# openai/robogym

Measured on AMD Instinct MI355X. Metric: env-steps/sec (whole node) dactyl/locked batch 8192; qpos L∞ vs MuJoCo (as restated by the in-repo CPU oracle: parity unpinned), higher is better.
Workload: dtype f32

## Files before the change

### robogym_amd/csrc/rg_kernel.h

```cpp
#ifndef RG_KERNEL_COMMON_H
#define RG_KERNEL_COMMON_H
#include "rg_types.h"

#ifdef RG_EMUL
#include "hip_emul.h"
#else
#include <hip/hip_runtime.h>
#endif

#ifdef RG_EMUL
typedef const RgModelDev& RgM;
#else
typedef const __attribute__((address_space(4))) RgModelDev& RgM;
#endif
#ifdef RG_FINE_PROF
#define RG_NPROF 56
#else
#define RG_NPROF 24
#endif
struct RgAux {
  const int *subtree_adr, *subtree;
  const uint32_t* dof_velmask;
};

// ... 446 lines not shown
    PFOR(d, m.nv) {
      float xf = 0;
      for (int b = 1; b < m.nbody; b++) {
        if (!in_chain(m, b, d)) continue;
        const float* w = P + RG_PRM_XFRC + 6 * b;
        v3 off = rg_xipos(m, s, b) - ld3(s.org + 3 * s.b2org[b]);
        xf += dot(ld3(w), jac_col(s, d, off)) + dot(ld3(w + 3), ld3(s.cdof + 6 * d));
      }
      s.qfrc_smooth[d] = xf;
    }
    SYNC();
  }
}


__device__ __forceinline__ bool seg_intersect(float p1x, float p1y, float p2x, float p2y, float p3x, float p3y, float p4x, float p4y) {
  float det = (p4y - p3y) * (p2x - p1x) - (p4x - p3x) * (p2y - p1y);
  if (fabsf(det) < 1e-15f) return false;
  float idet = rg_rcp(det);
  float a = ((p4x - p3x) * (p1y - p3y) - (p4y - p3y) * (p1x - p3x)) * idet;
  float b = ((p2x - p1x) * (p1y - p3y) - (p2y - p1y) * (p1x - p3x)) * idet;
  return a >= 0 && a <= 1 && b >= 0 && b <= 1;
}
__device__ __forceinline__ float wrap_circle(float* pnt, const float* d, bool has_sd, float sd0, float sd1, float rad) {
  float sq0 = d[0] * d[0] + d[1] * d[1], sq1 = d[2] * d[2] + d[3] * d[3], sqr = rad * rad;
  float dx = d[2] - d[0], dy = d[3] - d[1], dd = dx * dx + dy * dy;
  if (sq0 < sqr || sq1 < sqr || rad < 1e-15f || dd < 1e-15f) return -1;
  float a = clampf(-(dx * d[0] + dy * d[1]) * rg_rcp(dd), 0.f, 1.f);
  float nx = a * dx + d[0], ny = a * dy + d[1];
  if (nx * nx + ny * ny > sqr && (!has_sd || sd0 * nx + sd1 * ny >= 0)) return -1;
  float sol[2][4], good[2];
  float r0 = rg_sqrt(sq0 - sqr), r1 = rg_sqrt(sq1 - sqr), isq0 = rg_rcp(sq0), isq1 = rg_rcp(sq1);
  for (int i = 0; i < 2; i++) {
    float sgn = i == 0 ? 1.f : -1.f;
    sol[i][0] = (d[0] * sqr + sgn * rad * d[1] * r0) * isq0; sol[i][1] = (d[1] * sqr - sgn * rad * d[0] * r0) * isq0;
    sol[i][2] = (d[2] * sqr - sgn * rad * d[3] * r1) * isq1; sol[i][3] = (d[3] * sqr + sgn * rad * d[2] * r1) * isq1;
    if (has_sd) {
      float mx = sol[i][0] + sol[i][2], my = sol[i][1] + sol[i][3], n = fmaxf(rg_sqrt(mx * mx + my * my), 1e-15f);
      good[i] = (mx * sd0 + my * sd1) * rg_rcp(n);
    } else {
      float tx = sol[i][0] - sol[i][2], ty = sol[i][1] - sol[i][3];
      good[i] = -(tx * tx + ty * ty);
    }
    if (seg_intersect(d[0], d[1], sol[i][0], sol[i][1], d[2], d[3], sol[i][2], sol[i][3])) good[i] = -10000.f;
  }
  int k = good[0] > good[1] ? 0 : 1;
  for (int e = 0; e < 4; e++) pnt[e] = sol[k][e];
  if (seg_intersect(d[0], d[1], pnt[0], pnt[1], d[2], d[3], pnt[2], pnt[3])) return -1;
  return rad * acosf(clampf((pnt[0] * pnt[2] + pnt[1] * pnt[3]) * rg_rcp(sqr), -1.f, 1.f));
}
__device__ __forceinline__ float rg_wrap(v3& w0, v3& w1, v3 x0, v3 x1, v3 gpos, const float* gmat, float radius, int type, bool has_side, v3 side) {
  v3 p0 = mulmT(gmat, x0 - gpos), p1 = mulmT(gmat, x1 - gpos);
  if (norm(p0) < 1e-15f || norm(p1) < 1e-15f) return -1;
  v3 ax0, ax1;
  if (type == RG_WRAP_SPHERE) {
    ax0 = normalized(p0);
    v3 nrm = cross(p0, p1);
    if (norm(nrm) < 1e-15f) nrm = cross(ax0, fabsf(ax0.x) < 0.9f ? mk3(1, 0, 0) : mk3(0, 1, 0));
    nrm = normalized(nrm); ax1 = normalized(cross(nrm, ax0));
  } else { ax0 = mk3(1, 0, 0); ax1 = mk3(0, 1, 0); }
  float dd[4] = {dot(p0, ax0), dot(p0, ax1), dot(p1, ax0), dot(p1, ax1)}, sd0 = 0, sd1 = 0;
  if (has_side) {
    v3 sl = mulmT(gmat, side - gpos);
    sd0 = dot(sl, ax0); sd1 = dot(sl, ax1);
    float n = fmaxf(rg_sqrt(sd0 * sd0 + sd1 * sd1), 1e-15f), rn = radius * rg_rcp(n);
    sd0 *= rn; sd1 *= rn;
  }
  float pnt[4], wlen = wrap_circle(pnt, dd, has_side, sd0, sd1, radius);
  if (wlen < 0) return -1;
  v3 r0 = ax0 * pnt[0] + ax1 * pnt[1], r1 = ax0 * pnt[2] + ax1 * pnt[3];
  if (type == RG_WRAP_CYLINDER) {
    float L0 = rg_sqrt((dd[0] - pnt[0]) * (dd[0] - pnt[0]) + (dd[1] - pnt[1]) * (dd[1] - pnt[1]));
    float L1 = rg_sqrt((dd[2] - pnt[2]) * (dd[2] - pnt[2]) + (dd[3] - pnt[3]) * (dd[3] - pnt[3]));
    float iL = rg_rcp(L0 + wlen + L1);
    r0.z = p0.z + (p1.z - p0.z) * L0 * iL;
    r1.z = p0.z + (p1.z - p0.z) * (L0 + wlen) * iL;
    wlen = rg_sqrt(wlen * wlen + (r1.z - r0.z) * (r1.z - r0.z));
  }
  w0 = mulm(gmat, r0) + gpos; w1 = mulm(gmat, r1) + gpos;
  return wlen;
}

__device__ __forceinline__ void rg_tendon(RgM m, RgLds& s) {
  PFOR(t, m.ntendon) {
    int r0 = m.ten_path_adr[t], r1 = m.ten_path_adr[t + 1];
    const int* td = m.ten_dofs + 4 * t;
    int d0 = td[0], d1 = td[1], d2 = td[2], d3 = td[3];
    float J[4] = {0, 0, 0, 0}, L = 0;
    for (int r = r0; r < r1; r++) {
      const rgf4* R = (const rgf4*)m.ten_path + 2 * r;
      rgf4 ra = R[0], rb = R[1];
      int kind = __builtin_bit_cast(int, ra.x), w1 = __builtin_bit_cast(int, ra.y), w2 = __builtin_bit_cast(int, ra.z);
      if ((kind & 15) == 0) {
        float coef = ra.w;
        L += coef * s.qpos[w1];
        for (int e = 0; e < 4; e++) if (e == w2) J[e] += coef;
        continue;
      }
      float idiv = ra.w, radius = rb.x; int bits = __builtin_bit_cast(int, rb.y);
      int s0 = w1 & 255, s1 = (w1 >> 8) & 255, g = (w1 >> 16) & 255, sid = (w1 >> 24) & 255;
      int ba = w2 & 255, bs = (w2 >> 8) & 255, bg = (w2 >> 16) & 255;
      v3 pa = ld3(s.spos + 3 * s0), x1 = ld3(s.spos + 3 * s1), pb = x1, pc = mk3(0, 0, 0), pd = mk3(0, 0, 0);
      bool two = false;
      float wlen = -1;
      if ((kind & 15) == 2) {
        v3 w0 = mk3(0, 0, 0), w1p = mk3(0, 0, 0);
        float gm[9]; q2mat(gm, ldq(s.gquat + 4 * g));
        wlen = rg_wrap(w0, w1p, pa, x1, ld3(s.gpos + 3 * g), gm, radius, kind >> 4, sid != 255, sid != 255 ? ld3(s.spos + 3 * sid) : mk3(0, 0, 0));
        if (wlen >= 0) { pb = w0; pc = w1p; pd = x1; two = true; L += wlen * idiv; }
      }
      for (int seg = 0; seg < (two ? 2 : 1); seg++) {
        v3 q0 = seg ? pc : pa, q1 = seg ? pd : pb;
        int k0 = seg ? 2 : 0, k1 = two ? (seg ? 1 : 2) : 1;
        int b0 = seg ? bg : ba, b1 = two ? (seg ? bs : bg) : bs;
        v3 dif = q1 - q0;
        float dist = rg_sqrt(dot(dif, dif));
        L += dist * idiv;
        if (b0 != b1 && dist > 1e-15f) {
          dif = dif * rg_rcp(dist);
          v3 o0 = q0 - ld3(s.org + 3 * s.b2org[b0]), o1 = q1 - ld3(s.org + 3 * s.b2org[b1]);
          for (int e = 0; e < 4; e++) {
            int d = e == 0 ? d0 : (e == 1 ? d1 : (e == 2 ? d2 : d3));
            if (d < 0) continue;
            float v = 0;
            if ((bits >> (3 * e + k1)) & 1) v += dot(dif, jac_col(s, d, o1));
            if ((bits >> (3 * e + k0)) & 1) v -= dot(dif, jac_col(s, d, o0));
            J[e] += v * idiv;
          }
        }
      }
    }
    s.tenlen[t] = L;
    for (int e = 0; e < 4; e++) s.tenJ[4 * t + e] = J[e];
  }
  SYNC();
  PFOR(u, m.nu) {
    int id = m.actuator_trnid[u];
    s.actlen[u] = m.actuator_gear[u] * (m.actuator_trntype[u] == 0 ? s.qpos[m.jnt_qposadr[id]] : s.tenlen[id]);
  }
  SYNC();
}

__device__ __forceinline__ void rg_crb(RgM m, RgLds& s, const float* P, const int* subtree_adr, const int* subtree) {
  for (int w = LANE; w < m.nbody * 10; w += RG_WAVE) {
    int b = w / 10, k = w - 10 * b;
    float acc = 0;
    for (uint32_t bits = (uint32_t)m.subtree_mask[b]; bits; bits &= bits - 1) acc += s.cinert[10 * __builtin_ctz(bits) + k];
    s.crb[w] = acc;
  }
  SYNC();
  PFOR(e, m.nM) {
    const int ijb = m.M_ijb[e], i = ijb & 255, j = (ijb >> 8) & 255;
    float buf[6];
    mul_inert_vec(buf, s.crb + 10 * (ijb >> 16), s.cdof + 6 * i);
    const float* c = s.cdof + 6 * j;
    float v = c[0] * buf[0] + c[1] * buf[1] + c[2] * buf[2] + c[3] * buf[3] + c[4] * buf[4] + c[5] * buf[5];
    if (i == j) v += P[RG_PRM_DOF_ARMATURE + i];
    s.Msp[e] = v;
  }
  SYNC();
}
__device__ __forceinline__ void rg_M_to_blocks(RgM m, RgLds& s) {
  { rgf4 z; z.x = z.y = z.z = z.w = 0.f; rgf4* H4 = (rgf4*)s.H; for (int w = LANE; w < ((m.blkwords + 3) >> 2); w += RG_WAVE) H4[w] = z; }
  SYNC();
  PFOR(e, m.nM) { int a = m.M_ent[2 * e]; float v = s.Msp[e]; s.H[a & 0xFFFF] = v; s.H[(a >> 16) & 0xFFFF] = v; }
  SYNC();
}

struct SupPt { v3 v, s; };
struct MprGeom { int type; const float* quat; v3 pos; v3 size; int vertadr, nvert, mesh; float margin; float vscale = 1.f; };
struct MprEnv { const float* mesh_vert; const int* cell_adr; const rgf4 *cell_blk, *cell_ovf; float* prof; bool cells; bool plane_depth; };

__device__ __forceinline__ float vdot(v3 d, const rgf4& a) { return __builtin_fmaf(d.z, a.z, __builtin_fmaf(d.y, a.y, d.x * a.x)); }
template <int G> __device__ __forceinline__ void scan_batch(const rgf4* vert, int nvert, int base, v3 ld, float& bv, int& bi, v3& bp) {
  int i0 = base + (LANE & (G - 1)), last = nvert - 1;
  int j0 = i0 < last ? i0 : last, j1 = i0 + G < last ? i0 + G : last, j2 = i0 + 2 * G < last ? i0 + 2 * G : last, j3 = i0 + 3 * G < last ? i0 + 3 * G : last;
  rgf4 a = vert[j0], b = vert[j1], c = vert[j2], d = vert[j3];
  float da = vdot(ld, a), db = vdot(ld, b), dc = vdot(ld, c), dd = vdot(ld, d);
  if (da > bv) { bv = da; bi = j0; bp = mk3(a.x, a.y, a.z); }
  if (db > bv) { bv = db; bi = j1; bp = mk3(b.x, b.y, b.z); }
  if (dc > bv) { bv = dc; bi = j2; bp = mk3(c.x, c.y, c.z); }
  if (dd > bv) { bv = dd; bi = j3; bp = mk3(d.x, d.y, d.z); }
}
template <int G> __device__ __forceinline__ void scan_verts(const rgf4* vert, int nvert, v3 ld, float& bv, int& bi, v3& bp) {
  for (int base = 0; base < nvert; base += 4 * G) scan_batch<G>(vert, nvert, base, ld, bv, bi, bp);
}
__device__ __forceinline__ int dir_cell(v3 ld) {
  float ax = fabsf(ld.x), ay = fabsf(ld.y), az = fabsf(ld.z);
  int axis = ax >= ay ? (ax >= az ? 0 : 2) : (ay >= az ? 1 : 2);
  float mj = axis == 0 ? ld.x : (axis == 1 ? ld.y : ld.z), a = axis == 0 ? ld.y : (axis == 1 ? ld.z : ld.x), b = axis == 0 ? ld.z : (axis == 1 ? ld.x : ld.y);
  float inv = (0.5f * RG_CELLN) * rg_rcp(fmaxf(fabsf(mj), 1e-30f));
  int iu = (int)(a * inv + 0.5f * RG_CELLN), iv = (int)(b * inv + 0.5f * RG_CELLN);
  iu = iu < 0 ? 0 : (iu > RG_CELLN - 1 ? RG_CELLN - 1 : iu); iv = iv < 0 ? 0 : (iv > RG_CELLN - 1 ? RG_CELLN - 1 : iv);
  return ((2 * axis + (mj < 0 ? 1 : 0)) * RG_CELLN + iu) * RG_CELLN + iv;
}
template <int G> __device__ __forceinline__ void scan_cell(const int* celladr, const rgf4* cellblk, const rgf4* cellovf, v3 ld, float& bv, int& bi, v3& bp) {
  int cell = dir_cell(ld), l = LANE & (G - 1);
  int e = celladr[cell];
  if (G >= 4) {
    rgf4 a = cellblk[4 * cell + (l & 3)];
    float da = vdot(ld, a);
    if (da > bv) { bv = da; bi = __builtin_bit_cast(int, a.w); bp = mk3(a.x, a.y, a.z); }
  } else {
    rgf4 a = cellblk[4 * cell + 2 * (l & 1)], a2 = cellblk[4 * cell + 2 * (l & 1) + 1];
    float da = vdot(ld, a), da2 = vdot(ld, a2);
    if (da > bv) { bv = da; bi = __builtin_bit_cast(int, a.w); bp = mk3(a.x, a.y, a.z); }
    int i2 = __builtin_bit_cast(int, a2.w);
    if (da2 > bv || (da2 == bv && i2 < bi)) { bv = da2; bi = i2; bp = mk3(a2.x, a2.y, a2.z); }
  }
  int cnt = (e & 255) - 4, last = cnt - 1;
  if (cnt > 0) {
    const rgf4* rec = cellovf + (e >> 8);
    for (int base = 0; base < cnt; base += 2 * G) {
      int i0 = base + l, j0 = i0 < last ? i0 : last, j1 = i0 + G < last ? i0 + G : last;
      rgf4 b = rec[j0], c = rec[j1];
      float db = vdot(ld, b), dc = vdot(ld, c);
      int ib = __builtin_bit_cast(int, b.w), ic = __builtin_bit_cast(int, c.w);
      if (db > bv || (db == bv && ib < bi)) { bv = db; bi = ib; bp = mk3(b.x, b.y, b.z); }
      if (dc > bv || (dc == bv && ic < bi)) { bv = dc; bi = ic; bp = mk3(c.x, c.y, c.z); }
    }
  }
}
template <int G> __device__ __forceinline__ void scan_hull(const MprEnv& E, const MprGeom& g, v3 ld, float& bv, int& bi, v3& bp) {
  if (E.cells) scan_cell<G>(E.cell_adr + g.mesh * RG_NCELL, E.cell_blk + (size_t)g.mesh * (RG_NCELL * 4), E.cell_ovf, ld, bv, bi, bp);
  else scan_verts<G>((const rgf4*)E.mesh_vert + g.vertadr, g.nvert, ld, bv, bi, bp);
}
template <int G> __device__ __forceinline__ v3 pick_vert(float bv, int bi, v3 bp) {
  if (G == 64) {
    float vm = wave_max(bv);
    int wi = wave_min_i(bv == vm ? bi : 0x7fffffff);
    int wl = wave_min_i((bv == vm && bi == wi) ? LANE : 0x7fffffff);
    return mk3(lane_bcast(bp.x, wl), lane_bcast(bp.y, wl), lane_bcast(bp.z, wl));
  } else {
    float vm = grp_max<G>(bv);
    int wi = grp_min_i<G>(bv == vm ? bi : 0x7fffffff);
    bool win = bv == vm && bi == wi;
    return mk3(grp_max<G>(win ? bp.x : -3.0e38f), grp_max<G>(win ? bp.y : -3.0e38f), grp_max<G>(win ? bp.z : -3.0e38f));
  }
}
__device__ __forceinline__ v3 support_primitive(const MprGeom& g, v3 ld) {
// ... 496 lines not shown
        const float sc1 = (hdr & RG_PAIR_SCALED1) ? gscale : 1.f, sc2 = (hdr & RG_PAIR_SCALED2) ? gscale : 1.f;
        r3.z *= sc1; r3.w *= sc2;
        v3 p1 = ld3(s.gpos + 3 * g1), p2 = ld3(s.gpos + 3 * g2), dif = p2 - p1;
        isbb = ((hdr >> 20) & 255) == (RG_GEOM_BOX | (RG_GEOM_BOX << 4)); ispl = ((hdr >> 20) & 15) == RG_GEOM_PLANE;
        if (((hdr >> 20) & 15) == RG_GEOM_PLANE) {
          float d = dot(dif, qrot(ldq(s.gquat + 4 * g1), mk3(0, 0, 1))) - (r3.w + margin);
          hit = d <= 0; newlb = fmaxf(d, 0.f);
        } else {
          float d = sqrtf(dot(dif, dif)) - (r3.z + r3.w + margin);
          if (d <= 0) {
            float hm = 0.5f * margin + 1e-6f;
            v3 ea = mk3(r4.x * sc1 + hm, r4.y * sc1 + hm, r4.z * sc1 + hm), eb = mk3(r5.x * sc2 + hm, r5.y * sc2 + hm, r5.z * sc2 + hm);
            float Ra[9], Rb[9]; q2mat(Ra, ldq(s.gquat + 4 * g1)); q2mat(Rb, ldq(s.gquat + 4 * g2));
            float og = obb_gap(Ra, ea, Rb, eb, dif);
            hit = og < 0; newlb = fmaxf(og, 0.f);
          } else newlb = d;
        }
        if (pairlb) RG_ROW_ST(pairlb + q, fmaxf(newlb - 1e-6f, 0.f));
      }
      unsigned long long bal = __ballot(hit);
      bbany = bbany || (hit && isbb); plany = plany || (hit && ispl);
      int base = s.ncand;
      SYNC();
      if (hit) {
        int slot = base + __popcll(bal & ((1ull << LANE) - 1ull));
        if (slot < RG_MAXCAND) s.cand[slot] = q; else s.status |= RG_STATUS_CAND_FULL;
      }
      if (LANE == 0) { int n = base + __popcll(bal); s.ncand = n < RG_MAXCAND ? n : RG_MAXCAND; }
      SYNC();
    }
#ifdef RG_FINE_PROF
    if (prof && LANE == 0) prof[44] += (float)(rg_clock() - tref0);
#endif
    nt = 0;
  }
  if (prof && LANE == 0) prof[5] += (float)(rg_clock() - tb0);
  int ncand = s.ncand;
  if (LANE == 0) s.ncand2 = 0;
  SYNC();
  if (ncand > 16) rg_narrow_phase1<2>(c, ncand); else rg_narrow_phase1<4>(c, ncand);
  int ncand2 = s.ncand2;
  if (prof && LANE == 0) { prof[16] += (float)(rg_clock() - tb0); prof[17] += ncand; prof[18] += ncand2; }
  rg_narrow_phase2<4>(c, ncand2);
  if (prof && LANE == 0) prof[19] += (float)(rg_clock() - tb0);
  if (!(RG_L(c).flags & 16) && __ballot(bbany) != 0) rg_narrow_boxbox(c, ncand);
  if (__ballot(plany) != 0)
  for (int cbase = 0; cbase < ncand; cbase += RG_WAVE) {
  bool is_plane = false;
  if (cbase + LANE < ncand) is_plane = ((__builtin_bit_cast(int, m.pair_rec[RG_PAIRREC * s.cand[cbase + LANE]]) >> 20) & 15) == RG_GEOM_PLANE;
  unsigned long long plane_bits = __ballot(is_plane);
  while (plane_bits) {
    int ci = cbase + __builtin_ctzll(plane_bits); plane_bits &= plane_bits - 1;
    int p = s.cand[ci];
    int g1 = m.pair_geom[3 * p], g2 = m.pair_geom[3 * p + 1], dim = m.pair_geom[3 * p + 2];
    float margin = m.pair_prm[12 * p];
    int t2 = m.geom_type[g2];
    v3 p1 = ld3(s.gpos + 3 * g1), p2 = ld3(s.gpos + 3 * g2);
    MprGeom B;
    B.type = t2; B.quat = s.gquat + 4 * g2; B.size = ld3(m.geom_size + 3 * g2); B.margin = 0; B.mesh = -1; B.vertadr = 0; B.nvert = 0;
    if (__builtin_bit_cast(int, m.pair_rec[RG_PAIRREC * p]) & RG_PAIR_SCALED2) B.size = B.size * gscale;
    if (t2 == RG_GEOM_MESH) { B.mesh = m.geom_dataid[g2]; B.vertadr = m.mesh_vertadr[B.mesh]; B.nvert = m.mesh_vertnum[B.mesh]; }
    v3 n = qrot(ldq(s.gquat + 4 * g1), mk3(0, 0, 1));
    if (t2 == RG_GEOM_BOX) {
      int cnt = 0;
      for (int i = 0; i < 8 && cnt < 4; i++) {
        v3 lc = mk3((i & 1) ? B.size.x : -B.size.x, (i & 2) ? B.size.y : -B.size.y, (i & 4) ? B.size.z : -B.size.z);
        v3 c = qrot(ldq(B.quat), lc) + p2;
        float dist = dot(c - p1, n);
        if (dist > margin) continue;
        add_contact(s, p, dist, c - n * (0.5f * dist), n, dim); cnt++;
      }
    } else {
      B.pos = p2 - p1;
      v3 sp = rg_support<64>(rg_mpr_env(m, (float*)0, false), B, n * -1.0f);
      float dist = dot(sp, n);
      if (dist <= margin) add_contact(s, p, dist, sp + p1 - n * (0.5f * dist), n, dim);
    }
  }
  }
  SYNC();
}

__device__ __forceinline__ void rg_velocity(RgM m, RgLds& s, const float* P, const uint32_t* dof_velmask, const int* subtree_adr, const int* subtree) {
  PFOR(d, m.nv) {
    float cv[6] = {0, 0, 0, 0, 0, 0};
    for (int h = 0; h < 2; h++) {
      uint32_t bits = dof_velmask[2 * d + h];
      while (bits) { int a = __builtin_ctz(bits) + 32 * h; bits &= bits - 1; float q = s.qvel[a]; for (int e = 0; e < 6; e++) cv[e] += s.cdof[6 * a + e] * q; }
    }
    int j = m.dof_jntid[d];
    if (m.jnt_type[j] == RG_JNT_FREE && d - m.jnt_dofadr[j] < 3) { for (int e = 0; e < 6; e++) s.cdofdot[6 * d + e] = 0; }
    else cross_motion(s.cdofdot + 6 * d, cv, s.cdof + 6 * d);
  }
  PFOR(t, m.ntendon) {
    float v = 0;
    for (int e = 0; e < 4; e++) { int d = m.ten_dofs[4 * t + e]; if (d >= 0) v += s.tenJ[4 * t + e] * s.qvel[d]; }
    s.tenvel[t] = v;
    s.tenfrc[t] = m.tendon_stiffness[t] * (m.tendon_lengthspring[t] - s.tenlen[t]) - m.tendon_damping[t] * v;
  }
  SYNC();
  PFOR(k, m.body_geomnum[0]) s.gspeed[m.body_geomadr[0] + k] = 0;
  for (int b = 1 + LANE; b < m.nbody; b += RG_WAVE) {
    float cv[6] = {0, 0, 0, 0, 0, 0}, ca[6] = {0, 0, 0, -P[RG_PRM_GRAVITY], -P[RG_PRM_GRAVITY + 1], -P[RG_PRM_GRAVITY + 2]};
    for (int h = 0; h < 2; h++) {
      uint32_t bits = m.body_dofmask[2 * b + h];
      while (bits) {
        int a = __builtin_ctz(bits) + 32 * h; bits &= bits - 1; float q = s.qvel[a];
        for (int e = 0; e < 6; e++) { cv[e] += s.cdof[6 * a + e] * q; ca[e] += s.cdofdot[6 * a + e] * q; }
      }
    }
    {
      const float gsmax = fmaxf(P[RG_PRM_GEOM_SCALE], 1.f);
      v3 w = mk3(cv[0], cv[1], cv[2]), vo = mk3(cv[3], cv[4], cv[5]), og = ld3(s.org + 3 * s.b2org[b]);
      float wn = norm(w);
      int ga = m.body_geomadr[b], gn = m.body_geomnum[b];
      for (int k = 0; k < gn; k++) s.gspeed[ga + k] = norm(vo + cross(w, ld3(s.gpos + 3 * (ga + k)) - og)) + wn * (m.geom_rbound[ga + k] * gsmax);
    }
    float t1[6], t2[6], t3[6];
    mul_inert_vec(t1, s.cinert + 10 * b, ca);
    mul_inert_vec(t2, s.cinert + 10 * b, cv);
    cross_force(t3, cv, t2);
    for (int e = 0; e < 6; e++) s.cacc[6 * b + e] = t1[e] + t3[e];
  }
  SYNC();
  {
    float acc[(RG_MAXBODY * 6 + RG_WAVE - 1) / RG_WAVE];
#pragma unroll
    for (int k0 = 0; k0 < (RG_MAXBODY * 6 + RG_WAVE - 1) / RG_WAVE; k0++) {
      int w = LANE + RG_WAVE * k0, b = w / 6, k = w - 6 * b; float a = 0;
      if (w < m.nbody * 6 && b > 0) for (uint32_t bits = (uint32_t)m.subtree_mask[b]; bits; bits &= bits - 1) a += s.cacc[6 * __builtin_ctz(bits) + k];
      acc[k0] = a;
    }
    SYNC();
#pragma unroll
    for (int k0 = 0; k0 < (RG_MAXBODY * 6 + RG_WAVE - 1) / RG_WAVE; k0++) { int w = LANE + RG_WAVE * k0; if (w < m.nbody * 6) s.cacc[w] = acc[k0]; }
  }
  SYNC();
  PFOR(d, m.nv) {
    const rgf4 dr0 = ((const rgf4*)m.dof_rec)[2 * d]; const float spring_ref = m.dof_rec[8 * d + 4];
    const int w0 = __builtin_bit_cast(int, dr0.x);
    const float *c = s.cdof + 6 * d, *f = s.cacc + 6 * (w0 & 255);
    s.qfrc_bias[d] = c[0] * f[0] + c[1] * f[1] + c[2] * f[2] + c[3] * f[3] + c[4] * f[4] + c[5] * f[5];
    float pas = -P[RG_PRM_DOF_DAMPING + d] * s.qvel[d];
    if (dr0.z != 0) pas -= dr0.z * (s.qpos[__builtin_bit_cast(int, dr0.w)] - spring_ref);
    for (int q = (w0 >> 8) & 255; q < ((w0 >> 16) & 255); q++) { int tt = m.dof_ten[2 * q], sl = m.dof_ten[2 * q + 1]; pas += s.tenJ[4 * tt + sl] * s.tenfrc[tt]; }
    s.qfrc_passive[d] = pas;
  }
  SYNC();
}

static_assert(RG_MAXU <= RG_WAVE && RG_MAXNV <= RG_WAVE, "controller state / warm start: one lane per actuator / dof");
__device__ __forceinline__ void rg_pid(RgM m, RgLds& s, const float* P, float* st ) {
  float dt = P[RG_PRM_TIMESTEP];
  PFOR(u, m.nu) {
    const float* gp = P + RG_PRM_ACT_GAINPRM + 10 * u;
    float force;
    float lo = P[RG_PRM_ACT_FORCERANGE + 2 * u], hi = P[RG_PRM_ACT_FORCERANGE + 2 * u + 1];
    if (m.actuator_biastype[u] == 2) {
      float err = s.ctrl[u] - s.actlen[u];
      if (fabsf(err) < gp[5]) err = 0;
      float integ = clampf(st[0] + err * dt, -gp[2], gp[2]);
      float deriv = (1 - gp[4]) * st[2] + gp[4] * (err - st[1]) * rg_rcp(dt);
      force = gp[0] * (err + (gp[1] != 0 ? integ * rg_rcp(gp[1]) : 0.f) + gp[3] * deriv);
      st[0] = integ; st[1] = err; st[2] = deriv;
      if (lo != 0 || hi != 0) force = clampf(force, lo, hi);
    } else {
      float c = s.ctrl[u];
      if (m.actuator_ctrllimited[u]) c = clampf(c, P[RG_PRM_ACT_CTRLRANGE + 2 * u], P[RG_PRM_ACT_CTRLRANGE + 2 * u + 1]);
      force = gp[0] * c;
    }
    if (m.actuator_forcelimited[u]) force = clampf(force, lo, hi);
    s.actfrc[u] = force;
  }
  SYNC();
}
__device__ __forceinline__ void rg_smooth(RgM m, RgLds& s, const float* P) {
  PFOR(d, m.nv) {
    float f = 0;
    const int aw = __builtin_bit_cast(int, m.dof_rec[8 * d + 1]);
    for (int q = aw & 255; q < ((aw >> 8) & 255); q++) {
      int u = m.dof_act[2 * q], sl = m.dof_act[2 * q + 1];
      f += m.actuator_gear[u] * (sl < 0 ? 1.0f : s.tenJ[4 * m.actuator_trnid[u] + sl]) * s.actfrc[u];
    }
    s.qfrc_act[d] = f;
    float v = s.qfrc_passive[d] - s.qfrc_bias[d] + f + (s.has_xfrc ? s.qfrc_smooth[d] : 0.f);
    s.qfrc_smooth[d] = v; s.qacc_smooth[d] = v;
  }
  SYNC();
}

__device__ __forceinline__ float impedance(const float* si, float pos, float margin) {
  float dmin = clampf(si[0], 1e-4f, 0.9999f), dmax = clampf(si[1], 1e-4f, 0.9999f), width = fmaxf(si[2], 1e-15f);
  float mid = clampf(si[3], 1e-4f, 0.9999f), power = fmaxf(si[4], 1.0f);
  if (dmin == dmax || width <= 1e-15f) return 0.5f * (dmin + dmax);
  float x = fabsf((pos - margin) * rg_rcp(width));
  if (x >= 1) return dmax;
  if (x <= 0) return dmin;
  float y;
  if (power == 1) y = x;
  else if (power == 2) y = x <= mid ? x * x * rg_rcp(mid) : 1 - (1 - x) * (1 - x) * rg_rcp(1 - mid);
  else if (x <= mid) y = powf(x, power) / powf(mid, power - 1);
  else y = 1 - powf(1 - x, power) / powf(1 - mid, power - 1);
  return dmin + y * (dmax - dmin);
}
__device__ __forceinline__ void kb(float timestep, const float* solref, const float* solimp, float& K, float& B) {
  float dmax = clampf(solimp[1], 1e-4f, 0.9999f);
  if (solref[0] > 0) {
    float tc = fmaxf(solref[0], 2 * timestep), dr = solref[1];
    K = rg_rcp(fmaxf(1e-15f, dmax * dmax * tc * tc * dr * dr)); B = 2.0f * rg_rcp(fmaxf(1e-15f, dmax * tc));
  } else { K = -solref[0] / fmaxf(1e-15f, dmax * dmax); B = -solref[1] / fmaxf(1e-15f, dmax); }
}
__device__ __forceinline__ int nsrow(RgM m) { return m.nfric_dof + m.nfric_ten + 2 * m.nlim_jnt + 2 * m.nlim_ten; }
__device__ __forceinline__ void rg_build_row_desc(RgM m, RgLds& s) {
  int ns = nsrow(m);
  (void)ns;
  PFOR(w, m.ntendon * 4) { int d = m.ten_dofs[w]; s.ten_cdof[w] = (unsigned char)(d >= 0 ? m.d2c[d] : 255); }
  PFOR(i, m.nvc) { s.c2d[i] = (unsigned char)m.c2d[i]; s.cblk[i] = m.c_blk[i]; }
  PFOR(b, m.nbody) s.b2org[b] = (unsigned char)m.body_orgslot[b];
  SYNC();
}
template <bool FULL> __device__ __forceinline__ float srow_dot(const RgLds& s, int desc, const float* x) {
  int t = (desc >> 6) & 31; float v;
  if (t == 31) { int d = desc & 63; v = x[FULL ? s.c2d[d] : d]; }
  else { v = 0; for (int e = 0; e < 4; e++) { int d = s.ten_cdof[4 * t + e]; if (d != 255) v += s.tenJ[4 * t + e] * x[FULL ? s.c2d[d] : d]; } }
  return (desc >> 11) & 1 ? -v : v;
}
__device__ __forceinline__ void srow_scatter(RgLds& s, int desc, float coef, float* dst) {
  int t = (desc >> 6) & 31;
  if ((desc >> 11) & 1) coef = -coef;
  if (t == 31) { atomicAdd(dst + (desc & 63), coef); return; }
  for (int e = 0; e < 4; e++) { int d = s.ten_cdof[4 * t + e]; if (d != 255) atomicAdd(dst + d, coef * s.tenJ[4 * t + e]); }
}
__device__ __forceinline__ void srow_hess(RgM m, RgLds& s, int desc, float D) {
  int t = (desc >> 6) & 31;
  if (t == 31) { int d = desc & 63; atomicAdd(s.H + d * m.hs + d, D); return; }
  for (int a = 0; a < 4; a++) { int da = s.ten_cdof[4 * t + a]; if (da == 255) continue;
    for (int b = 0; b < 4; b++) { int db = s.ten_cdof[4 * t + b]; if (db == 255 || db > da) continue; atomicAdd(s.H + da * m.hs + db, D * s.tenJ[4 * t + a] * s.tenJ[4 * t + b]); } }
}
__device__ __forceinline__ void srow_hess_tree(RgLds& s, int desc, float D) {
  int t = (desc >> 6) & 31;
  if (t == 31) { int d = desc & 63, blk = s.cblk[d]; atomicAdd(s.H + (blk & 0xFFFF) + d - ((blk >> 16) & 255), D); return; }
  for (int a = 0; a < 4; a++) { int da = s.ten_cdof[4 * t + a]; if (da == 255) continue;
    int blk = s.cblk[da];
    for (int b = 0; b < 4; b++) { int db = s.ten_cdof[4 * t + b]; if (db == 255 || db > da) continue; atomicAdd(s.H + (blk & 0xFFFF) + db - ((blk >> 16) & 255), D * s.tenJ[4 * t + a] * s.tenJ[4 * t + b]); } }
}
__device__ __forceinline__ int npyr(int dim) { return dim == 1 ? 1 : 2 * (dim - 1); }
__device__ __forceinline__ int nbasis(int dim) { return dim >= 4 ? 4 : (dim == 1 ? 1 : 3); }

__device__ __forceinline__ void rg_make_constraint(RgM m, RgLds& s, const float* P) {
  int ncon = s.ncon;
  PFOR(c, ncon) {
    const float* R = m.pair_rec + RG_PAIRREC * s.c_pair[c];
    s.c_nnz[c] = __popc(__builtin_bit_cast(uint32_t, R[23])) + __popc(__builtin_bit_cast(uint32_t, R[24]));
  }
  SYNC();
  {
    int c = LANE, off = 0, sz = 0;
    if (c < ncon) { for (int q = 0; q < c; q++) off += nbasis(s.c_dim[q]) * s.c_nnz[q]; sz = nbasis(s.c_dim[c]) * s.c_nnz[c]; s.c_off[c] = off; }
#if defined(RG_CAP_HIST) && !defined(RG_EMUL)
    if (ncon > 0 && c == ncon - 1) { atomicAdd(rg_cap_hist + (ncon < 63 ? ncon : 63), 1u); const int bin = (off + sz) >> 4; atomicAdd(rg_cap_hist + 64 + (bin < 127 ? bin : 127), 1u); }
    if (ncon == 0 && c == 0) { atomicAdd(rg_cap_hist, 1u); atomicAdd(rg_cap_hist + 64, 1u); }
#endif
    int firstbad = wave_min_i((c < ncon && off + sz > RG_CPOOL) ? c : 0x7fffffff);
    if (firstbad < ncon) { ncon = firstbad; if (LANE == 0) { s.ncon = ncon; s.status |= RG_STATUS_CON_FULL; } }
  }
  SYNC();
  for (int w = LANE; w < ncon * RG_W; w += RG_WAVE) {
    int c = w / RG_W, sl = w - c * RG_W, p = s.c_pair[c], nnz = s.c_nnz[c];
    if (sl >= nnz) continue;
    const float* R = m.pair_rec + RG_PAIRREC * p;
    int bb = __builtin_bit_cast(int, R[19]), b1 = bb & 255, b2 = bb >> 8;
    uint32_t lo = __builtin_bit_cast(uint32_t, R[23]), hi = __builtin_bit_cast(uint32_t, R[24]);
    int k = sl; uint32_t bits = lo; int base = 0;
    if (k >= __popc(lo)) { k -= __popc(lo); bits = hi; base = 32; }
    for (int q = 0; q < k; q++) bits &= bits - 1;
    int d = base + __builtin_ctz(bits);
    v3 pos = ld3(s.c_pos + 3 * c);
    v3 jp = mk3(0, 0, 0), jr = mk3(0, 0, 0);
    if (in_chain(m, b2, d)) { jp = jp + jac_col(s, d, pos - ld3(s.org + 3 * s.b2org[b2])); jr = jr + ld3(s.cdof + 6 * d); }
    if (in_chain(m, b1, d)) { jp = jp - jac_col(s, d, pos - ld3(s.org + 3 * s.b2org[b1])); jr = jr - ld3(s.cdof + 6 * d); }
    float f[9]; st3(f, ld3(s.c_normal + 3 * c)); make_frame(f);
    s.c_idx[c * RG_W + sl] = (unsigned char)m.d2c[d];
    float* Bc = s.c_pool + s.c_off[c]; int nb = nbasis(s.c_dim[c]);
    Bc[sl] = dot(ld3(f), jp);
    if (nb >= 3) { Bc[nnz + sl] = dot(ld3(f + 3), jp); Bc[2 * nnz + sl] = dot(ld3(f + 6), jp); }
    if (nb >= 4) Bc[3 * nnz + sl] = dot(ld3(f), jr);
  }
  SYNC();
  PFOR(c, ncon) {
    int p = s.c_pair[c], dim = s.c_dim[c];
    const float* prm = m.pair_prm + 12 * p;
    const int hdr = __builtin_bit_cast(int, m.pair_rec[RG_PAIRREC * p]), bb = __builtin_bit_cast(int, m.pair_rec[RG_PAIRREC * p + 19]), b1 = bb & 255, b2 = bb >> 8;
    float tran = P[RG_PRM_BODY_INVWEIGHT0 + 2 * b1] + P[RG_PRM_BODY_INVWEIGHT0 + 2 * b2];
    float includemargin = prm[0] - prm[1], dist = s.c_dist[c];
    const int pg1 = hdr & 255, pg2 = (hdr >> 8) & 255;
    const float mix = m.pair_mix[p];
    const float* r1 = P + RG_PRM_GEOM_SOLREF + 2 * pg1; const float* r2 = P + RG_PRM_GEOM_SOLREF + 2 * pg2;
    const float* i1 = P + RG_PRM_GEOM_SOLIMP + 5 * pg1; const float* i2 = P + RG_PRM_GEOM_SOLIMP + 5 * pg2;
    float solref[2], solimp[5];
    if (r1[0] > 0 && r2[0] > 0) { solref[0] = mix * r1[0] + (1.f - mix) * r2[0]; solref[1] = mix * r1[1] + (1.f - mix) * r2[1]; }
    else { solref[0] = fminf(r1[0], r2[0]); solref[1] = fminf(r1[1], r2[1]); }
    for (int q = 0; q < 5; q++) solimp[q] = mix * i1[q] + (1.f - mix) * i2[q];
    float imp = impedance(solimp, dist, includemargin), K, B;
    kb(P[RG_PRM_TIMESTEP], solref, solimp, K, B);
    const float fr_slide = fmaxf(P[RG_PRM_GEOM_FRICTION + 3 * pg1], P[RG_PRM_GEOM_FRICTION + 3 * pg2]), fr_spin = fmaxf(P[RG_PRM_GEOM_FRICTION + 3 * pg1 + 1], P[RG_PRM_GEOM_FRICTION + 3 * pg2 + 1]);
    float mu0 = fr_slide;
    float R;
    if (dim == 1) R = fmaxf(1e-15f, (1 - imp) * tran * rg_rcp(imp));
    else { float Rf = fmaxf(1e-15f, (1 - imp) * (tran + mu0 * mu0 * tran) * rg_rcp(imp)); float mu = mu0 * rg_rsqrt(m.impratio); R = 2 * mu * mu * Rf; }
    s.c_D[c] = rg_rcp(R);
    s.c_mu[2 * c] = fr_slide; s.c_mu[2 * c + 1] = fr_spin;
    s.c_aref0[c] = -K * imp * (dist - includemargin); s.c_kb[c] = B;
  }
  SYNC();
}

#define RG_RSLOTS ((RG_MAXSROW + RG_WAVE - 1) / RG_WAVE)
struct RowRegs { int desc[RG_RSLOTS]; float D[RG_RSLOTS], aref[RG_RSLOTS], floss[RG_RSLOTS], jar[RG_RSLOTS], jv[RG_RSLOTS]; int quad[RG_RSLOTS]; float pjar[RG_PSLOTS], pjv[RG_PSLOTS], paref[RG_PSLOTS]; };
__device__ __forceinline__ float srow_force(float D, float f, float x) {
  if (!(D > 0)) return 0.f;
  if (f > 0) { float R = rg_rcp(D); return x <= -R * f ? f : (x >= R * f ? -f : -D * x); }
  return x < 0 ? -D * x : 0.f;
}
__device__ __forceinline__ void rg_static_rows(RgM m, const RgLds& s, const float* P, RowRegs& R) {
  int ns = nsrow(m);
#pragma unroll
  for (int k = 0; k < RG_RSLOTS; k++) {
    int r = LANE + RG_WAVE * k;
    if (r >= ns) { R.D[k] = 0.f; R.aref[k] = 0.f; R.floss[k] = 0.f; R.desc[k] = 0; continue; }
    const rgf4* S = (const rgf4*)m.srow_rec + 4 * r;
    const rgf4 sa = S[0], sb = S[1], sc = S[2], sd = S[3];
    const int w0 = __builtin_bit_cast(int, sa.x), kind = w0 >> 16, desc = w0 & 0xFFFF, src = __builtin_bit_cast(int, sa.y), ofl = __builtin_bit_cast(int, sa.w);
    const bool fric = kind < 2;
    const float diag = P[__builtin_bit_cast(int, sa.z)];
    const float floss = kind == 0 ? P[ofl] : sb.x;
    const float solref[2] = {sb.w, sc.x}, solimp[5] = {sc.y, sc.z, sc.w, sd.x, sd.y};
    float pos = 0, margin = 0; bool active = true;
    if (!fric) {
      const float x = kind == 2 ? s.qpos[src] : s.tenlen[src], bound = P[__builtin_bit_cast(int, sb.y)];
      pos = (desc >> 11) & 1 ? bound - x : x - bound;
      margin = kind == 2 ? P[__builtin_bit_cast(int, sb.z)] : sb.z; active = pos < margin;
    }
    R.desc[k] = desc;
    float D = 0, aref = 0;
    if (active) {
      float imp = impedance(solimp, pos, margin), K, B;
      float R = fmaxf(1e-15f, (1 - imp) * diag * rg_rcp(imp));
      kb(P[RG_PRM_TIMESTEP], solref, solimp, K, B);
      if (fric) K = 0;
      float vel = srow_dot<true>(s, desc, s.qvel);
      D = rg_rcp(R); aref = -B * vel - K * imp * (pos - margin);
    }
    R.D[k] = D; R.aref[k] = aref; R.floss[k] = fric ? floss : 0.f;
  }
}
template <bool SROWS = true> __device__ __forceinline__ void rg_J_mul(RgM m, RgLds& s, RowRegs& R, const float* x, bool to_jv) {
  int ns = nsrow(m), ncon = s.ncon;
#pragma unroll
  for (int k = 0; k < (SROWS ? RG_RSLOTS : 0); k++) {
    int r = LANE + RG_WAVE * k;
    if (r < ns && R.D[k] > 0) { float v = srow_dot<false>(s, R.desc[k], x); if (to_jv) R.jv[k] = v; else R.jar[k] = v - R.aref[k]; }
  }
  for (int c0 = 0; c0 < ncon; c0 += 4) {
    const int c = c0 + (LANE >> 4), sl = LANE & 15, cc = c < ncon ? c : c0;
    const int nnz = s.c_nnz[cc], nb = nbasis(s.c_dim[cc]);
    const bool on = c < ncon && sl < nnz;
    const int slc = on ? sl : 0;
    const float* Bc = s.c_pool + s.c_off[cc] + slc;
    const float xv = on ? x[s.c_idx[cc * RG_W + slc]] : 0.f;
    float p0 = Bc[0] * xv, p1 = nb > 1 ? Bc[nnz] * xv : 0.f, p2 = nb > 2 ? Bc[2 * nnz] * xv : 0.f, p3 = nb > 3 ? Bc[3 * nnz] * xv : 0.f;
    p0 = grp_sum16(p0); p1 = grp_sum16(p1); p2 = grp_sum16(p2); p3 = grp_sum16(p3);
    if (c < ncon && sl < 4) s.c_bdot[4 * c + sl] = sl == 0 ? p0 : (sl == 1 ? p1 : (sl == 2 ? p2 : p3));
  }
  SYNC();
#pragma unroll
  for (int kk = 0; kk < RG_PSLOTS; kk++) {
    int w = LANE + RG_WAVE * kk;
    if (w >= ncon * 6) continue;
    int c = w / 6, q = w - 6 * c, dim = s.c_dim[c];
    if (q >= npyr(dim)) continue;
    float v;
    if (dim == 1) v = s.c_bdot[4 * c];
    else { int k = q >> 1; float mu = s.c_mu[2 * c + (k >> 1)]; v = s.c_bdot[4 * c] + ((q & 1) ? -mu : mu) * s.c_bdot[4 * c + k + 1]; }
    if (to_jv) R.pjv[kk] = v; else R.pjar[kk] = v - R.paref[kk];
  }
  SYNC();
}
__device__ __forceinline__ float rg_constraint_update(RgM m, RgLds& s, RowRegs& R, bool& changed, int& nset) {
// ... 1461 lines not shown
```

Before: 2.092 million.

## Hoist model-constant loads and batch masked LDS gathers in tendon, CRB and velocity stages

Model-constant reads (tendon path addresses, actuator ids, subtree masks, M_ijb, armature, dof records, body masks, geom rbounds) are loaded into registers at stage entry, before the SYNC-separated phases that use them, so their latency overlaps earlier work. Masked subtree sums and velocity accumulations are unrolled into batches of 4 or 8 independent LDS loads to expose memory-level parallelism. Tendon path records are software-prefetched one iteration ahead, and the PID and contact-parameter loads are grouped up front. In exchange it raises register pressure, which may reduce occupancy. It also replaces the strided loops with one lane per item, which relies on new static_asserts that the counts fit in a wave.

```diff
diff --git a/robogym_amd/csrc/rg_kernel.h b/robogym_amd/csrc/rg_kernel.h
--- a/robogym_amd/csrc/rg_kernel.h
+++ b/robogym_amd/csrc/rg_kernel.h
@@ -552,14 +552,23 @@
 }
 
 __device__ __forceinline__ void rg_tendon(RgM m, RgLds& s) {
+  int a_id = 0, a_type = 1, a_qadr = 0; float a_gear = 0;
+  if (LANE < m.nu) { a_id = m.actuator_trnid[LANE]; a_type = m.actuator_trntype[LANE]; a_gear = m.actuator_gear[LANE]; }
+  int p_r0 = 0, p_r1 = 0, p_d0 = -1, p_d1 = -1, p_d2 = -1, p_d3 = -1;
+  if (LANE < m.ntendon) {
+    p_r0 = m.ten_path_adr[LANE]; p_r1 = m.ten_path_adr[LANE + 1];
+    const int* td = m.ten_dofs + 4 * LANE; p_d0 = td[0]; p_d1 = td[1]; p_d2 = td[2]; p_d3 = td[3];
+  }
+  if (LANE < m.nu && a_type == 0) a_qadr = m.jnt_qposadr[a_id];
   PFOR(t, m.ntendon) {
-    int r0 = m.ten_path_adr[t], r1 = m.ten_path_adr[t + 1];
-    const int* td = m.ten_dofs + 4 * t;
-    int d0 = td[0], d1 = td[1], d2 = td[2], d3 = td[3];
+    int r0 = p_r0, r1 = p_r1;
+    int d0 = p_d0, d1 = p_d1, d2 = p_d2, d3 = p_d3;
     float J[4] = {0, 0, 0, 0}, L = 0;
+    rgf4 na, nb; na.x = na.y = na.z = na.w = 0.f; nb = na;
+    if (r0 < r1) { const rgf4* R = (const rgf4*)m.ten_path + 2 * r0; na = R[0]; nb = R[1]; }
     for (int r = r0; r < r1; r++) {
-      const rgf4* R = (const rgf4*)m.ten_path + 2 * r;
-      rgf4 ra = R[0], rb = R[1];
+      const rgf4 ra = na, rb = nb;
+      if (r + 1 < r1) { const rgf4* R = (const rgf4*)m.ten_path + 2 * (r + 1); na = R[0]; nb = R[1]; }
       int kind = __builtin_bit_cast(int, ra.x), w1 = __builtin_bit_cast(int, ra.y), w2 = __builtin_bit_cast(int, ra.z);
       if ((kind & 15) == 0) {
         float coef = ra.w;
@@ -604,28 +613,52 @@
     for (int e = 0; e < 4; e++) s.tenJ[4 * t + e] = J[e];
   }
   SYNC();
-  PFOR(u, m.nu) {
-    int id = m.actuator_trnid[u];
-    s.actlen[u] = m.actuator_gear[u] * (m.actuator_trntype[u] == 0 ? s.qpos[m.jnt_qposadr[id]] : s.tenlen[id]);
-  }
-  SYNC();
-}
-
+  static_assert(RG_MAXU <= RG_WAVE && RG_MAXTEN <= RG_WAVE, "tendon stage: one lane per tendon / actuator");
+  PFOR(u, m.nu) s.actlen[u] = a_gear * (a_type == 0 ? s.qpos[a_qadr] : s.tenlen[a_id]);
+  SYNC();
+}
+
+template <int STRIDE> __device__ __forceinline__ float rg_mask_sum(const float* base, uint32_t bits) {
+  float acc = 0;
+  while (bits) {
+    float v[8];
+#pragma unroll
+    for (int i = 0; i < 8; i++) { const float x = base[STRIDE * (bits ? __builtin_ctz(bits) : 0)]; v[i] = bits ? x : 0.f; bits &= bits - 1; }
+#pragma unroll
+    for (int i = 0; i < 8; i++) acc += v[i];
+  }
+  return acc;
+}
 __device__ __forceinline__ void rg_crb(RgM m, RgLds& s, const float* P, const int* subtree_adr, const int* subtree) {
-  for (int w = LANE; w < m.nbody * 10; w += RG_WAVE) {
-    int b = w / 10, k = w - 10 * b;
-    float acc = 0;
-    for (uint32_t bits = (uint32_t)m.subtree_mask[b]; bits; bits &= bits - 1) acc += s.cinert[10 * __builtin_ctz(bits) + k];
-    s.crb[w] = acc;
-  }
-  SYNC();
-  PFOR(e, m.nM) {
-    const int ijb = m.M_ijb[e], i = ijb & 255, j = (ijb >> 8) & 255;
+  constexpr int NE = (RG_MAXNM + RG_WAVE - 1) / RG_WAVE;
+  const int nM = m.nM;
+  int ijb[NE]; float arm[NE];
+  {
+    constexpr int NR = (RG_MAXBODY * 10 + RG_WAVE - 1) / RG_WAVE;
+    const int n = m.nbody * 10;
+    uint32_t mask[NR];
+#pragma unroll
+    for (int r = 0; r < NR; r++) { const int w = LANE + RG_WAVE * r; mask[r] = w < n ? (uint32_t)m.subtree_mask[w / 10] : 0u; }
+#pragma unroll
+    for (int r = 0; r < NE; r++) { const int e = LANE + RG_WAVE * r; ijb[r] = e < nM ? m.M_ijb[e] : 0x0100; }
+#pragma unroll
+    for (int r = 0; r < NE; r++) { const int i = ijb[r] & 255, j = (ijb[r] >> 8) & 255; arm[r] = i == j ? P[RG_PRM_DOF_ARMATURE + i] : 0.f; }
+#pragma unroll
+    for (int r = 0; r < NR; r++) {
+      const int w = LANE + RG_WAVE * r, b = w / 10, k = w - 10 * b;
+      if (w < n) s.crb[w] = rg_mask_sum<10>(s.cinert + k, mask[r]);
+    }
+  }
+  SYNC();
+#pragma unroll
+  for (int r = 0; r < NE; r++) {
+    const int e = LANE + RG_WAVE * r, i = ijb[r] & 255, j = (ijb[r] >> 8) & 255;
+    if (e >= nM) continue;
     float buf[6];
-    mul_inert_vec(buf, s.crb + 10 * (ijb >> 16), s.cdof + 6 * i);
+    mul_inert_vec(buf, s.crb + 10 * (ijb[r] >> 16), s.cdof + 6 * i);
     const float* c = s.cdof + 6 * j;
     float v = c[0] * buf[0] + c[1] * buf[1] + c[2] * buf[2] + c[3] * buf[3] + c[4] * buf[4] + c[5] * buf[5];
-    if (i == j) v += P[RG_PRM_DOF_ARMATURE + i];
+    if (i == j) v += arm[r];
     s.Msp[e] = v;
   }
   SYNC();
@@ -1288,39 +1321,85 @@
 }
 
 __device__ __forceinline__ void rg_velocity(RgM m, RgLds& s, const float* P, const uint32_t* dof_velmask, const int* subtree_adr, const int* subtree) {
-  PFOR(d, m.nv) {
+  static_assert(RG_MAXNV <= RG_WAVE && RG_MAXTEN <= RG_WAVE && RG_MAXBODY <= RG_WAVE, "velocity stage: one lane per dof / tendon / body");
+  constexpr int NSUB = (RG_MAXBODY * 6 + RG_WAVE - 1) / RG_WAVE, NRB = 4 , NDT = 2 ;
+  const int nv = m.nv, nt = m.ntendon, nb = m.nbody, d = LANE, t = LANE, b = 1 + LANE;
+  int dj = 0; uint32_t vm[2] = {0u, 0u}; rgf4 dr0; dr0.x = dr0.y = dr0.z = dr0.w = 0.f; float spring_ref = 0, damping = 0;
+  if (d < nv) {
+    dj = m.dof_jntid[d]; dr0 = ((const rgf4*)m.dof_rec)[2 * d]; spring_ref = m.dof_rec[8 * d + 4];
+    vm[0] = dof_velmask[2 * d]; vm[1] = dof_velmask[2 * d + 1]; damping = P[RG_PRM_DOF_DAMPING + d];
+  }
+  int td[4] = {-1, -1, -1, -1}; float t_stiff = 0, t_spring = 0, t_damp = 0;
+  if (t < nt) {
+    for (int e = 0; e < 4; e++) td[e] = m.ten_dofs[4 * t + e];
+    t_stiff = m.tendon_stiffness[t]; t_spring = m.tendon_lengthspring[t]; t_damp = m.tendon_damping[t];
+  }
+  uint32_t bm[2] = {0u, 0u}; int ga = 0, gn = 0;
+  if (b < nb) { bm[0] = m.body_dofmask[2 * b]; bm[1] = m.body_dofmask[2 * b + 1]; ga = m.body_geomadr[b]; gn = m.body_geomnum[b]; }
+  uint32_t sub[NSUB];
+#pragma unroll
+  for (int k0 = 0; k0 < NSUB; k0++) { const int w = LANE + RG_WAVE * k0, sb = w / 6; sub[k0] = (w < nb * 6 && sb > 0) ? (uint32_t)m.subtree_mask[sb] : 0u; }
+  const int g0a = m.body_geomadr[0], g0n = m.body_geomnum[0];
+  const float grav0 = P[RG_PRM_GRAVITY], grav1 = P[RG_PRM_GRAVITY + 1], grav2 = P[RG_PRM_GRAVITY + 2], gsmax = fmaxf(P[RG_PRM_GEOM_SCALE], 1.f);
+  int jt = 0, jda = 0, dten[2 * NDT]; const int w0 = __builtin_bit_cast(int, dr0.x), tq0 = (w0 >> 8) & 255, tq1 = (w0 >> 16) & 255;
+#pragma unroll
+  for (int i = 0; i < 2 * NDT; i++) dten[i] = 0;
+  if (d < nv) {
+    jt = m.jnt_type[dj]; jda = m.jnt_dofadr[dj];
+#pragma unroll
+    for (int i = 0; i < NDT; i++) if (tq0 + i < tq1) { dten[2 * i] = m.dof_ten[2 * (tq0 + i)]; dten[2 * i + 1] = m.dof_ten[2 * (tq0 + i) + 1]; }
+  }
+  float rbound[NRB];
+#pragma unroll
+  for (int k = 0; k < NRB; k++) rbound[k] = k < gn ? m.geom_rbound[ga + k] : 0.f;
+
+  if (d < nv) {
     float cv[6] = {0, 0, 0, 0, 0, 0};
     for (int h = 0; h < 2; h++) {
-      uint32_t bits = dof_velmask[2 * d + h];
-      while (bits) { int a = __builtin_ctz(bits) + 32 * h; bits &= bits - 1; float q = s.qvel[a]; for (int e = 0; e < 6; e++) cv[e] += s.cdof[6 * a + e] * q; }
-    }
-    int j = m.dof_jntid[d];
-    if (m.jnt_type[j] == RG_JNT_FREE && d - m.jnt_dofadr[j] < 3) { for (int e = 0; e < 6; e++) s.cdofdot[6 * d + e] = 0; }
+      uint32_t bits = vm[h];
+      while (bits) {
+        float q[4], c[4][6]; bool on[4];
+#pragma unroll
+        for (int i = 0; i < 4; i++) {
+          on[i] = bits != 0; const int a = on[i] ? __builtin_ctz(bits) + 32 * h : 0; bits &= bits - 1;
+          q[i] = s.qvel[a]; for (int e = 0; e < 6; e++) c[i][e] = s.cdof[6 * a + e];
+        }
+#pragma unroll
+        for (int i = 0; i < 4; i++) if (on[i]) for (int e = 0; e < 6; e++) cv[e] += c[i][e] * q[i];
+      }
+    }
+    if (jt == RG_JNT_FREE && d - jda < 3) { for (int e = 0; e < 6; e++) s.cdofdot[6 * d + e] = 0; }
     else cross_motion(s.cdofdot + 6 * d, cv, s.cdof + 6 * d);
   }
-  PFOR(t, m.ntendon) {
+  if (t < nt) {
     float v = 0;
-    for (int e = 0; e < 4; e++) { int d = m.ten_dofs[4 * t + e]; if (d >= 0) v += s.tenJ[4 * t + e] * s.qvel[d]; }
+    for (int e = 0; e < 4; e++) { int dd = td[e]; if (dd >= 0) v += s.tenJ[4 * t + e] * s.qvel[dd]; }
     s.tenvel[t] = v;
-    s.tenfrc[t] = m.tendon_stiffness[t] * (m.tendon_lengthspring[t] - s.tenlen[t]) - m.tendon_damping[t] * v;
-  }
-  SYNC();
-  PFOR(k, m.body_geomnum[0]) s.gspeed[m.body_geomadr[0] + k] = 0;
-  for (int b = 1 + LANE; b < m.nbody; b += RG_WAVE) {
-    float cv[6] = {0, 0, 0, 0, 0, 0}, ca[6] = {0, 0, 0, -P[RG_PRM_GRAVITY], -P[RG_PRM_GRAVITY + 1], -P[RG_PRM_GRAVITY + 2]};
+    s.tenfrc[t] = t_stiff * (t_spring - s.tenlen[t]) - t_damp * v;
+  }
+  SYNC();
+  PFOR(k, g0n) s.gspeed[g0a + k] = 0;
+  if (b < nb) {
+    float cv[6] = {0, 0, 0, 0, 0, 0}, ca[6] = {0, 0, 0, -grav0, -grav1, -grav2};
     for (int h = 0; h < 2; h++) {
-      uint32_t bits = m.body_dofmask[2 * b + h];
+      uint32_t bits = bm[h];
       while (bits) {
-        int a = __builtin_ctz(bits) + 32 * h; bits &= bits - 1; float q = s.qvel[a];
-        for (int e = 0; e < 6; e++) { cv[e] += s.cdof[6 * a + e] * q; ca[e] += s.cdofdot[6 * a + e] * q; }
+        float q[2], c[2][6], cd[2][6]; bool on[2];
+#pragma unroll
+        for (int i = 0; i < 2; i++) {
+          on[i] = bits != 0; const int a = on[i] ? __builtin_ctz(bits) + 32 * h : 0; bits &= bits - 1;
+          q[i] = s.qvel[a]; for (int e = 0; e < 6; e++) { c[i][e] = s.cdof[6 * a + e]; cd[i][e] = s.cdofdot[6 * a + e]; }
+        }
+#pragma unroll
+        for (int i = 0; i < 2; i++) if (on[i]) for (int e = 0; e < 6; e++) { cv[e] += c[i][e] * q[i]; ca[e] += cd[i][e] * q[i]; }
       }
     }
     {
-      const float gsmax = fmaxf(P[RG_PRM_GEOM_SCALE], 1.f);
       v3 w = mk3(cv[0], cv[1], cv[2]), vo = mk3(cv[3], cv[4], cv[5]), og = ld3(s.org + 3 * s.b2org[b]);
       float wn = norm(w);
-      int ga = m.body_geomadr[b], gn = m.body_geomnum[b];
-      for (int k = 0; k < gn; k++) s.gspeed[ga + k] = norm(vo + cross(w, ld3(s.gpos + 3 * (ga + k)) - og)) + wn * (m.geom_rbound[ga + k] * gsmax);
+#pragma unroll
+      for (int k = 0; k < NRB; k++) if (k < gn) s.gspeed[ga + k] = norm(vo + cross(w, ld3(s.gpos + 3 * (ga + k)) - og)) + wn * (rbound[k] * gsmax);
+      for (int k = NRB; k < gn; k++) s.gspeed[ga + k] = norm(vo + cross(w, ld3(s.gpos + 3 * (ga + k)) - og)) + wn * (m.geom_rbound[ga + k] * gsmax);
     }
     float t1[6], t2[6], t3[6];
     mul_inert_vec(t1, s.cinert + 10 * b, ca);
@@ -1330,26 +1409,25 @@
   }
   SYNC();
   {
-    float acc[(RG_MAXBODY * 6 + RG_WAVE - 1) / RG_WAVE];
-#pragma unroll
-    for (int k0 = 0; k0 < (RG_MAXBODY * 6 + RG_WAVE - 1) / RG_WAVE; k0++) {
-      int w = LANE + RG_WAVE * k0, b = w / 6, k = w - 6 * b; float a = 0;
-      if (w < m.nbody * 6 && b > 0) for (uint32_t bits = (uint32_t)m.subtree_mask[b]; bits; bits &= bits - 1) a += s.cacc[6 * __builtin_ctz(bits) + k];
-      acc[k0] = a;
+    float acc[NSUB];
+#pragma unroll
+    for (int k0 = 0; k0 < NSUB; k0++) {
+      const int w = LANE + RG_WAVE * k0, sb = w / 6, k = w - 6 * sb;
+      acc[k0] = rg_mask_sum<6>(s.cacc + k, sub[k0]);
     }
     SYNC();
 #pragma unroll
-    for (int k0 = 0; k0 < (RG_MAXBODY * 6 + RG_WAVE - 1) / RG_WAVE; k0++) { int w = LANE + RG_WAVE * k0; if (w < m.nbody * 6) s.cacc[w] = acc[k0]; }
-  }
-  SYNC();
-  PFOR(d, m.nv) {
-    const rgf4 dr0 = ((const rgf4*)m.dof_rec)[2 * d]; const float spring_ref = m.dof_rec[8 * d + 4];
-    const int w0 = __builtin_bit_cast(int, dr0.x);
+    for (int k0 = 0; k0 < NSUB; k0++) { int w = LANE + RG_WAVE * k0; if (w < nb * 6) s.cacc[w] = acc[k0]; }
+  }
+  SYNC();
+  if (d < nv) {
     const float *c = s.cdof + 6 * d, *f = s.cacc + 6 * (w0 & 255);
     s.qfrc_bias[d] = c[0] * f[0] + c[1] * f[1] + c[2] * f[2] + c[3] * f[3] + c[4] * f[4] + c[5] * f[5];
-    float pas = -P[RG_PRM_DOF_DAMPING + d] * s.qvel[d];
+    float pas = -damping * s.qvel[d];
     if (dr0.z != 0) pas -= dr0.z * (s.qpos[__builtin_bit_cast(int, dr0.w)] - spring_ref);
-    for (int q = (w0 >> 8) & 255; q < ((w0 >> 16) & 255); q++) { int tt = m.dof_ten[2 * q], sl = m.dof_ten[2 * q + 1]; pas += s.tenJ[4 * tt + sl] * s.tenfrc[tt]; }
+#pragma unroll
+    for (int i = 0; i < NDT; i++) if (tq0 + i < tq1) pas += s.tenJ[4 * dten[2 * i] + dten[2 * i + 1]] * s.tenfrc[dten[2 * i]];
+    for (int q = tq0 + NDT; q < tq1; q++) { int tt = m.dof_ten[2 * q], sl = m.dof_ten[2 * q + 1]; pas += s.tenJ[4 * tt + sl] * s.tenfrc[tt]; }
     s.qfrc_passive[d] = pas;
   }
   SYNC();
@@ -1359,10 +1437,13 @@
 __device__ __forceinline__ void rg_pid(RgM m, RgLds& s, const float* P, float* st ) {
   float dt = P[RG_PRM_TIMESTEP];
   PFOR(u, m.nu) {
-    const float* gp = P + RG_PRM_ACT_GAINPRM + 10 * u;
+    float gp[6];
+    for (int i = 0; i < 6; i++) gp[i] = P[RG_PRM_ACT_GAINPRM + 10 * u + i];
     float force;
     float lo = P[RG_PRM_ACT_FORCERANGE + 2 * u], hi = P[RG_PRM_ACT_FORCERANGE + 2 * u + 1];
-    if (m.actuator_biastype[u] == 2) {
+    const float clo = P[RG_PRM_ACT_CTRLRANGE + 2 * u], chi = P[RG_PRM_ACT_CTRLRANGE + 2 * u + 1];
+    const int biastype = m.actuator_biastype[u], ctrllimited = m.actuator_ctrllimited[u], forcelimited = m.actuator_forcelimited[u];
+    if (biastype == 2) {
       float err = s.ctrl[u] - s.actlen[u];
       if (fabsf(err) < gp[5]) err = 0;
       float integ = clampf(st[0] + err * dt, -gp[2], gp[2]);
@@ -1372,10 +1453,10 @@
       if (lo != 0 || hi != 0) force = clampf(force, lo, hi);
     } else {
       float c = s.ctrl[u];
-      if (m.actuator_ctrllimited[u]) c = clampf(c, P[RG_PRM_ACT_CTRLRANGE + 2 * u], P[RG_PRM_ACT_CTRLRANGE + 2 * u + 1]);
+      if (ctrllimited) c = clampf(c, clo, chi);
       force = gp[0] * c;
     }
-    if (m.actuator_forcelimited[u]) force = clampf(force, lo, hi);
+    if (forcelimited) force = clampf(force, lo, hi);
     s.actfrc[u] = force;
   }
   SYNC();
@@ -1481,12 +1562,13 @@
     if (k >= __popc(lo)) { k -= __popc(lo); bits = hi; base = 32; }
     for (int q = 0; q < k; q++) bits &= bits - 1;
     int d = base + __builtin_ctz(bits);
+    const uint32_t ch2 = m.body_dofmask[2 * b2 + (d >> 5)], ch1 = m.body_dofmask[2 * b1 + (d >> 5)]; const int cd = m.d2c[d];
     v3 pos = ld3(s.c_pos + 3 * c);
     v3 jp = mk3(0, 0, 0), jr = mk3(0, 0, 0);
-    if (in_chain(m, b2, d)) { jp = jp + jac_col(s, d, pos - ld3(s.org + 3 * s.b2org[b2])); jr = jr + ld3(s.cdof + 6 * d); }
-    if (in_chain(m, b1, d)) { jp = jp - jac_col(s, d, pos - ld3(s.org + 3 * s.b2org[b1])); jr = jr - ld3(s.cdof + 6 * d); }
+    if ((ch2 >> (d & 31)) & 1u) { jp = jp + jac_col(s, d, pos - ld3(s.org + 3 * s.b2org[b2])); jr = jr + ld3(s.cdof + 6 * d); }
+    if ((ch1 >> (d & 31)) & 1u) { jp = jp - jac_col(s, d, pos - ld3(s.org + 3 * s.b2org[b1])); jr = jr - ld3(s.cdof + 6 * d); }
     float f[9]; st3(f, ld3(s.c_normal + 3 * c)); make_frame(f);
-    s.c_idx[c * RG_W + sl] = (unsigned char)m.d2c[d];
+    s.c_idx[c * RG_W + sl] = (unsigned char)cd;
     float* Bc = s.c_pool + s.c_off[c]; int nb = nbasis(s.c_dim[c]);
     Bc[sl] = dot(ld3(f), jp);
     if (nb >= 3) { Bc[nnz + sl] = dot(ld3(f + 3), jp); Bc[2 * nnz + sl] = dot(ld3(f + 6), jp); }
@@ -1501,15 +1583,17 @@
     float includemargin = prm[0] - prm[1], dist = s.c_dist[c];
     const int pg1 = hdr & 255, pg2 = (hdr >> 8) & 255;
     const float mix = m.pair_mix[p];
-    const float* r1 = P + RG_PRM_GEOM_SOLREF + 2 * pg1; const float* r2 = P + RG_PRM_GEOM_SOLREF + 2 * pg2;
-    const float* i1 = P + RG_PRM_GEOM_SOLIMP + 5 * pg1; const float* i2 = P + RG_PRM_GEOM_SOLIMP + 5 * pg2;
+    float r1[2], r2[2], i1[5], i2[5];
+    for (int q = 0; q < 2; q++) { r1[q] = P[RG_PRM_GEOM_SOLREF + 2 * pg1 + q]; r2[q] = P[RG_PRM_GEOM_SOLREF + 2 * pg2 + q]; }
+    for (int q = 0; q < 5; q++) { i1[q] = P[RG_PRM_GEOM_SOLIMP + 5 * pg1 + q]; i2[q] = P[RG_PRM_GEOM_SOLIMP + 5 * pg2 + q]; }
+    const float fr_slide = fmaxf(P[RG_PRM_GEOM_FRICTION + 3 * pg1], P[RG_PRM_GEOM_FRICTION + 3 * pg2]), fr_spin = fmaxf(P[RG_PRM_GEOM_FRICTION + 3 * pg1 + 1], P[RG_PRM_GEOM_FRICTION + 3 * pg2 + 1]);
+    const float timestep = P[RG_PRM_TIMESTEP];
     float solref[2], solimp[5];
     if (r1[0] > 0 && r2[0] > 0) { solref[0] = mix * r1[0] + (1.f - mix) * r2[0]; solref[1] = mix * r1[1] + (1.f - mix) * r2[1]; }
     else { solref[0] = fminf(r1[0], r2[0]); solref[1] = fminf(r1[1], r2[1]); }
     for (int q = 0; q < 5; q++) solimp[q] = mix * i1[q] + (1.f - mix) * i2[q];
     float imp = impedance(solimp, dist, includemargin), K, B;
-    kb(P[RG_PRM_TIMESTEP], solref, solimp, K, B);
-    const float fr_slide = fmaxf(P[RG_PRM_GEOM_FRICTION + 3 * pg1], P[RG_PRM_GEOM_FRICTION + 3 * pg2]), fr_spin = fmaxf(P[RG_PRM_GEOM_FRICTION + 3 * pg1 + 1], P[RG_PRM_GEOM_FRICTION + 3 * pg2 + 1]);
+    kb(timestep, solref, solimp, K, B);
     float mu0 = fr_slide;
     float R;
     if (dim == 1) R = fmaxf(1e-15f, (1 - imp) * tran * rg_rcp(imp));
```

Result: faster. 2.156 million (median of 6 runs) (+3.1%).
